# weifengliu-ssslab/Benchmark_SpMV_using_CSR5

Hardware: AMD Instinct MI355X
Metric: fp64 SpMV GFLOPS (higher is better)
Workload: dtype f64

## Files before the change

benchmark_spmv_using_csr5_amd/csrc/csr5_capi.hip:

```cpp
#include <algorithm>
#include <chrono>
#include <cstdio>
#include <cstdlib>
#include <cstring>
#include <string>
#include <unordered_map>
#include <vector>

#include "csr5_internal.h"

using namespace csr5;

namespace {

thread_local std::string g_last_error;

}

namespace csr5 {
void set_last_error(const std::string &msg) { g_last_error = msg; }
}

namespace {

// ... 668 lines not shown
    if (rc != CSR5HIP_SUCCESS)
        return rc;
    Geometry &g = h->g;
    hipStream_t s = h->stream;

    double t0 = now_ms();
    rc = reserve_aux(h);
    if (rc != CSR5HIP_SUCCESS)
        return rc;
    h->t_malloc += now_ms() - t0;

    if (g.p > 0) {
        rc = build_format_arrays(h);
        if (rc != CSR5HIP_SUCCESS)
            return rc;
        if (h->is_child && h->hot_enabled)
            HIP_TRY(launch_transpose_values(g, h->d, h->value_type, s));
        else
            HIP_TRY(launch_transpose(g, h->d, h->value_type, true, s));
        auto finish = [&]() -> int {
            return derive_kernel_tables(h);
        };
        rc = finish();
        if (rc != CSR5HIP_SUCCESS) {
            const std::string why = g_last_error;
            if (h->is_child && h->hot_enabled)
                h->format = -1;
            else if (launch_transpose(g, h->d, h->value_type, false, s) != hipSuccess ||
                     hipStreamSynchronize(s) != hipSuccess)
                h->format = -1;
            g_last_error = why;
            return rc;
        }
// ... 219 lines not shown
        if (!hot && auto_count) {
            if (h->hot_cover_pct >= HOT_AUTO_MIN_COVER_PCT) {
                h->t_slab = now_ms() - t0;
                return CSR5HIP_SUCCESS;
            }
            S = S_plain;
        }
    }
    int bits = 0;
    while ((1 << bits) < S)
        bits++;

    HIP_TRY(h->b_col2.reserve((size_t)g.nnz * 4));
    HIP_TRY(h->b_val2.reserve((size_t)g.nnz * h->vsize()));
    HIP_TRY(slab_partition(g, h->d, h->value_type, S, bits, h->slab_shift, (uint32_t *)t.hist, t.scan_tmp, scan_bytes,
                           (int32_t *)h->b_col2.ptr, h->b_val2.ptr, (uint32_t *)t.key, s));
    HIP_TRY(slab_count_segments(g.nnz, (const uint32_t *)t.key, t.sel_tmp, (unsigned int *)t.count, s));
    unsigned int m2 = 0;
    HIP_TRY(hipMemcpyAsync(&m2, t.count, 4, hipMemcpyDeviceToHost, s));
    HIP_TRY(hipStreamSynchronize(s));
    HIP_TRY(h->b_row_ptr2.reserve(((size_t)m2 + 1) * 4));
    HIP_TRY(h->b_rowidx.reserve((size_t)m2 + 1));
    HIP_TRY(slab_segments(g.nnz, (const uint32_t *)t.key, t.sel_tmp, (int32_t *)h->b_row_ptr2.ptr, (unsigned char *)h->b_rowidx.ptr, s));
    HIP_TRY(h->b_base.reserve(slab_base_words(g.m, S) * 4));
    HIP_TRY(h->b_nonempty.reserve(((size_t)g.m / 32 + 16) * 4));
    HIP_TRY(slab_tables(g.m, (int)m2, g.nnz, S, g.p, h->d.row_ptr, (int32_t *)h->b_row_ptr2.ptr, (const uint32_t *)t.key,
                        (const uint32_t *)t.hist, (uint32_t *)h->b_base.ptr, (uint32_t *)h->b_nonempty.ptr, s));
    HIP_TRY(h->b_P.reserve(((size_t)m2 + 1) * h->vsize()));
    HIP_TRY(hipMemsetAsync(h->b_P.ptr, 0, ((size_t)m2 + 1) * h->vsize(), s));

    if (hot) {
        HIP_TRY(slab_hot_finish(S, g.p, hot_p, hot_T, g.nnz, hot_capacity, (const uint32_t *)t.hist,
                                (int32_t *)h->b_hot_count.ptr, (int32_t *)h->b_hot_tile0.ptr, (int32_t *)h->b_slab_off.ptr, s));
        std::vector<int32_t> first_tile((size_t)S + 1);
        HIP_TRY(hipMemcpyAsync(first_tile.data(), h->b_hot_tile0.ptr, ((size_t)S + 1) * 4, hipMemcpyDeviceToHost, s));
        HIP_TRY(hipStreamSynchronize(s));
        const int rounds = S / NUM_XCD;
        std::vector<int> by_size((size_t)S), order((size_t)S, 0), used(NUM_XCD, 0);
// ... 2 lines not shown
            by_size[k] = k;
        std::stable_sort(by_size.begin(), by_size.end(), [&](int a, int b) {
            return first_tile[a + 1] - first_tile[a] > first_tile[b + 1] - first_tile[b];
        });
        for (int k : by_size) {
            int best = -1;
            for (int x = 0; x < NUM_XCD; x++)
                if (used[x] < rounds && (best < 0 || load[x] < load[best]))
                    best = x;
            order[(size_t)best * rounds + used[best]++] = k;
            load[best] += first_tile[k + 1] - first_tile[k];
        }
        HIP_TRY(hipMemcpyAsync((int32_t *)h->b_hot_tile0.ptr + S + 1, order.data(), (size_t)S * 4, hipMemcpyHostToDevice, s));
        int32_t cold_total = 0;
        {
            HIP_TRY(h->b_col_lo.reserve((size_t)g.nnz * 2 + 64));
            HIP_TRY(h->b_col_hi.reserve((size_t)g.nnz + 64));
            const size_t cold_cap = std::min(cold_words, (size_t)g.nnz);
            HIP_TRY(h->b_cold_base.reserve(((size_t)S + 1) * 4));
            HIP_TRY(h->b_cold_cols.reserve((cold_cap + 1) * 4));
            HIP_TRY(h->b_xperm.reserve(((size_t)S * hot_capacity + cold_cap + (size_t)hot_T + 1) * h->vsize()));
            HIP_TRY(hipMemsetAsync(tb + o_ref, 0, cold_words, s));
            HIP_TRY(slab_hot_pack(g.n, g.nnz, hot_T, hot_p, S, bits, h->slab_shift, (const int32_t *)h->b_slab_off.ptr, ht.hotmap,
                                  (const uint32_t *)ht.cnt, (const uint32_t *)t.key, (int32_t *)h->b_col2.ptr, (uint16_t *)h->b_col_lo.ptr,
                                  (uint8_t *)h->b_col_hi.ptr, (uint8_t *)(tb + o_ref), (uint32_t *)(tb + o_rank),
                                  (uint32_t *)(tb + o_keys), (uint32_t *)(tb + o_keys2),
                                  (uint32_t *)(tb + o_src), tb + o_sort, cold_sort_bytes, (int32_t *)h->b_cold_base.ptr,
                                  (int32_t *)h->b_cold_cols.ptr, s));
            HIP_TRY(hipMemcpyAsync(&cold_total, (int32_t *)h->b_cold_base.ptr + S, 4, hipMemcpyDeviceToHost, s));
        }
        HIP_TRY(hipStreamSynchronize(s));
        h->cold_total = cold_total;
    }
    HIP_TRY(hipStreamSynchronize(s));

    csr5hip_handle c = h->slab_child ? h->slab_child : new csr5hip_handle_s();
    h->slab_child = c;
    c->is_child = true;
    c->g.m = (int)m2;
// ... 720 lines not shown
    return CSR5HIP_SUCCESS;
}

int csr5hip_timer_stop(csr5hip_handle h, double *ms)
{
    if (!h || !ms || !h->ev0)
        return CSR5HIP_INVALID_ARGUMENT;
    HIP_TRY(hipEventRecord(h->ev1, h->stream));
    HIP_TRY(hipEventSynchronize(h->ev1));
    float f = 0;
    HIP_TRY(hipEventElapsedTime(&f, h->ev0, h->ev1));
    *ms = f;
    return CSR5HIP_SUCCESS;
}

}
```

benchmark_spmv_using_csr5_amd/csrc/csr5_format.hip:

```cpp
#include "csr5_internal.h"

#include <rocprim/device/device_scan.hpp>

namespace csr5 {

__device__ __forceinline__ int upper_bound(const int32_t *__restrict__ a, int key, int size)
{
    int lo = 0, hi = size;
    while (lo < hi) {
        int mid = (int)(((unsigned)lo + (unsigned)hi) >> 1);
        if (a[mid] <= key)
            lo = mid + 1;
        else
            hi = mid;
    }
    return lo;
}

__device__ __forceinline__ void stamp_phase(uint32_t *__restrict__ counters, int slot)
{
    if (counters && blockIdx.x == 0 && threadIdx.x == 0)
        *reinterpret_cast<unsigned long long *>(counters + STAMP_WORD + 2 * slot) = wall_clock64();
}

// ... 607 lines not shown
        hipLaunchKernelGGL(k_offset_scan_small, dim3(1), dim3(1024), 0, s, d.offset_ptr, g.p + 1);
        return hipGetLastError();
    }
    return rocprim::exclusive_scan(tmp, tmp_bytes, d.offset_ptr, d.offset_ptr, 0, (size_t)g.p + 1, rocprim::plus<int32_t>(), s);
}

hipError_t launch_desc_offset(const Geometry &g, const DeviceArrays &d, hipStream_t s)
{
    if (g.p <= 1)
        return hipSuccess;
    hipLaunchKernelGGL(k_desc_offset, dim3(div_up(g.p - 1, FMT_WAVES_PER_BLOCK)), dim3(FMT_BLOCK), 0, s, g,
                       d.row_ptr, d.tile_ptr, d.tile_desc, d.offset_ptr, d.offset);
    return hipGetLastError();
}

template <typename VT, int SIGMA>
__global__ void __launch_bounds__(FMT_BLOCK) k_transpose_values(Geometry g, VT *__restrict__ val, uint32_t *__restrict__ counters)
{
    stamp_phase(counters, 2);
    constexpr int T = OMEGA * SIGMA;
    const int lane = threadIdx.x & (OMEGA - 1);
    const int t = blockIdx.x * FMT_WAVES_PER_BLOCK + (threadIdx.x >> 6);
    if (t >= g.p - 1)
        return;
    VT *tile = val + (size_t)t * T;
    VT v[SIGMA];
    constexpr int PER = 16 / sizeof(VT);
    typedef VT piece_t __attribute__((ext_vector_type(PER)));
    static_assert(SIGMA % PER == 0, "whole 16-byte pieces per lane");
#pragma unroll
    for (int q = 0; q < SIGMA / PER; q++) {
        const piece_t w = *reinterpret_cast<const piece_t *>(tile + lane * SIGMA + q * PER);
#pragma unroll
        for (int e = 0; e < PER; e++)
            v[q * PER + e] = w[e];
    }
    asm volatile("s_waitcnt vmcnt(0)" ::: "memory");
#pragma unroll
    for (int q = 0; q < SIGMA / PER; q++) {
        piece_t w;
#pragma unroll
        for (int e = 0; e < PER; e++)
            w[e] = v[q * PER + e];
        *reinterpret_cast<piece_t *>(tile + ((size_t)q * OMEGA + lane) * PER) = w;
    }
}

hipError_t launch_transpose(const Geometry &g, const DeviceArrays &d, int value_type, bool r2c, hipStream_t s)
{
    if (g.p <= 1)
        return hipSuccess;
    const size_t vsz = value_type == CSR5HIP_F64 ? 8 : 4;
    int tpb = (int)(12288 / ((size_t)g.tile_elems * (vsz + 4)));
    tpb = tpb < 1 ? 1 : (tpb > 16 ? 16 : tpb);
    const size_t lds = (size_t)tpb * g.sigma * transpose_pitch(g.sigma) * (vsz + 4);
    const dim3 grid((unsigned)((g.p - 1 + tpb - 1) / tpb));
    if (value_type == CSR5HIP_F64)
        hipLaunchKernelGGL(k_transpose<double>, grid, dim3(FMT_BLOCK), lds, s, g, d.tile_ptr, d.col, (double *)d.val, r2c ? 1 : 0, tpb,
                           r2c ? d.counters : nullptr);
    else
        hipLaunchKernelGGL(k_transpose<float>, grid, dim3(FMT_BLOCK), lds, s, g, d.tile_ptr, d.col, (float *)d.val, r2c ? 1 : 0, tpb,
                           r2c ? d.counters : nullptr);
    return hipGetLastError();
}

hipError_t launch_transpose_values(const Geometry &g, const DeviceArrays &d, int value_type, hipStream_t s)
{
    if (g.p <= 1)
        return hipSuccess;
    const dim3 grid((unsigned)div_up(g.p - 1, FMT_WAVES_PER_BLOCK)), block(FMT_BLOCK);
#define CSR5_TV(VT, S)                                                                                                \
    hipLaunchKernelGGL((k_transpose_values<VT, S>), grid, block, 0, s, g, (VT *)d.val, d.counters);                  \
    return hipGetLastError();
    if (value_type == CSR5HIP_F64) {
        switch (g.sigma) {
        case 8: CSR5_TV(double, 8)
        case 16: CSR5_TV(double, 16)
        }
    } else {
        switch (g.sigma) {
        case 8: CSR5_TV(float, 8)
        case 16: CSR5_TV(float, 16)
        }
    }
#undef CSR5_TV
    return hipErrorInvalidValue;
}

hipError_t launch_tile_tables(const Geometry &g, const DeviceArrays &d, int value_size, uint32_t *host_words, bool export_only,
                              hipStream_t s)
{
    if (g.p <= 0)
        return hipSuccess;
    if (export_only) {
        hipLaunchKernelGGL(k_stats_export, dim3(1), dim3(1024), 0, s, g, d.tile_ptr, d.tile_hdr, d.offset_ptr, d.counters,
                           host_words, 1);
        return hipGetLastError();
    }
    hipLaunchKernelGGL(k_tile_tables, dim3(div_up(g.p, FMT_WAVES_PER_BLOCK)), dim3(FMT_BLOCK), 0, s, g, d.row_ptr,
                       d.tile_ptr, d.col, reinterpret_cast<uint4 *>(d.carry_meta), d.tile_hdr, d.counters,
                       xwin_elems(value_size), value_size == 8 ? 4 : 5);
    hipError_t e = hipGetLastError();
    if (e != hipSuccess)
// ... 25 lines not shown
```

benchmark_spmv_using_csr5_amd/csrc/csr5_internal.h:

```cpp
#pragma once

#include <hip/hip_runtime.h>
#include <stdint.h>

#include "csr5hip.h"

namespace csr5 {

constexpr int OMEGA = CSR5HIP_OMEGA;
#ifndef CSR5_WAVES_PER_BLOCK
#define CSR5_WAVES_PER_BLOCK 1
#endif
constexpr int WAVES_PER_BLOCK = CSR5_WAVES_PER_BLOCK;
constexpr int BLOCK = OMEGA * WAVES_PER_BLOCK;
constexpr int FMT_WAVES_PER_BLOCK = 2;
constexpr int FMT_BLOCK = OMEGA * FMT_WAVES_PER_BLOCK;
constexpr int BIT_SS = 6;
constexpr uint32_t ROW_MASK = 0x7FFFFFFFu;
constexpr int STAMP_WORD = 8;
constexpr int COUNTER_WORDS = 16;
constexpr int NUM_XCD = 8;
constexpr int RUN_SERIAL_MAX = 64;
#ifndef CSR5_XWIN_BYTES
#define CSR5_XWIN_BYTES 4096
// ... 49 lines not shown
    const int32_t *cold_cols;
    int cold_total;
    const float *val32;
    const uint32_t *col16;
    const int32_t *base16;
    const uint32_t *col31;
};

hipError_t launch_row_scan(const Geometry &g, const DeviceArrays &d, hipStream_t s);
hipError_t launch_tile_desc(const Geometry &g, const DeviceArrays &d, hipStream_t s);
size_t offset_scan_tmp_bytes(int entries);
hipError_t launch_offset_scan(const Geometry &g, const DeviceArrays &d, void *tmp, size_t tmp_bytes, hipStream_t s);
hipError_t launch_desc_offset(const Geometry &g, const DeviceArrays &d, hipStream_t s);
hipError_t launch_transpose(const Geometry &g, const DeviceArrays &d, int value_type, bool r2c,
                            hipStream_t s);
hipError_t launch_transpose_values(const Geometry &g, const DeviceArrays &d, int value_type, hipStream_t s);
hipError_t launch_tile_tables(const Geometry &g, const DeviceArrays &d, int value_size, uint32_t *host_words, bool export_only,
                              hipStream_t s);
hipError_t launch_col16(const Geometry &g, const DeviceArrays &d, uint32_t *col16, int32_t *base16, uint32_t *wide_tiles,
                        hipStream_t s);
constexpr int COL16_SPAN = 32768;
constexpr bool col16_sigma(int sigma) { return sigma == 8 || sigma == 12 || sigma == 16 || sigma == 24 || sigma == 32; }
hipError_t launch_col31(const Geometry &g, const DeviceArrays &d, uint32_t *col31, hipStream_t s);
constexpr bool col31_sigma(int sigma) { return sigma >= 4 && sigma <= 8; }
hipError_t launch_warmup(hipStream_t s);
hipError_t launch_validate_csr(int m, int n, int nnz, const int32_t *row_ptr, const int32_t *col, uint32_t *flag,
                               hipStream_t s);

hipError_t slab_scan_tmp_bytes(size_t items, size_t *bytes);
hipError_t slab_select_tmp_bytes(int nnz, size_t *bytes);
hipError_t slab_partition(const Geometry &g, const DeviceArrays &d, int value_type, int S, int bits, int shift,
                          uint32_t *hist, void *scan_tmp, size_t scan_tmp_bytes, int32_t *col2, void *val2,
                          uint32_t *key2, hipStream_t s);
hipError_t slab_count_segments(int nnz, const uint32_t *key2, void *tmp, unsigned int *d_count, hipStream_t s);
hipError_t slab_segments(int nnz, const uint32_t *key2, const void *tmp, int32_t *row_ptr2, unsigned char *rowidx, hipStream_t s);
size_t slab_base_words(int m, int S);
hipError_t slab_tables(int m, int m2, int nnz, int S, int p, const int32_t *row_ptr, int32_t *row_ptr2, const uint32_t *key2,
                       const uint32_t *chunk_start, uint32_t *base, uint32_t *nonempty, hipStream_t s);
hipError_t slab_hot_select(int n, int nnz, int S, int bits, int shift, int capacity, int min_count, int sample_stride,
                           const int32_t *col, uint32_t *cnt, void *hotmap, uint32_t *chist, uint32_t *thr,
                           int32_t *hot_cols, int32_t *hot_count, unsigned long long *covered, hipStream_t s);
hipError_t slab_hot_finish(int S, int p_hist, int p, int T, int nnz, int capacity, const uint32_t *chunk_start,
                           int32_t *hot_count, int32_t *tile0, int32_t *slab_off, hipStream_t s);
size_t slab_cold_words(int n, int S, int bits, int shift);
hipError_t slab_cold_sort_tmp_bytes(size_t total, int slab_bits, size_t *bytes);
hipError_t slab_hot_pack(int n, int nnz, int T, int p, int S, int bits, int shift, const int32_t *slab_off, const void *hotmap,
                         const uint32_t *cnt, const uint32_t *key2, int32_t *col2, uint16_t *col_lo, uint8_t *col_hi, uint8_t *ref, uint32_t *rank_of,
                         uint32_t *keys, uint32_t *keys_sorted, uint32_t *src_sorted, void *sort_tmp, size_t sort_tmp_bytes,
                         int32_t *cold_base, int32_t *cold_cols, hipStream_t s);
size_t slab_local_columns(int n, int bits, int shift);
size_t slab_hotmap_bytes(int n, int S, int bits, int shift);
int slab_hot_buckets();
hipError_t launch_slab_combine(int m, int tail_start, int zero_empty, int S, int value_type, const uint32_t *base,
                               const unsigned char *rowidx, const uint32_t *nonempty, const void *P, int segments, void *y,
                               hipStream_t s);

struct SpmvOptions {
    int mode;
    int xcd_remap;
    int x_window;
    int lds_y;
    int stream_nt;
// ... 48 lines not shown
```

benchmark_spmv_using_csr5_amd/csrc/csr5_slab.hip:

```cpp
#include "csr5_internal.h"
#include "csr5_slabmap.h"

#include <rocprim/device/device_radix_sort.hpp>
#include <rocprim/device/device_scan.hpp>
#include <rocprim/iterator/counting_iterator.hpp>

namespace csr5 {

constexpr int SLAB_BLOCK = 256;
constexpr int SLAB_MAX = 64;
constexpr uint32_t SLAB_KEY_FIRST = 0x80000000u;

__host__ __device__ inline size_t slab_hot_groups(int n, int shift, int bits) { return (slab_local_count(n, shift, bits) + 127) / 128; }
__device__ __forceinline__ bool hot_lookup(const uint4 w, uint32_t bit, uint32_t &below)
{
    const unsigned long long lo = (unsigned long long)w.x | ((unsigned long long)w.y << 32);
    const unsigned long long hi = (unsigned long long)w.z | ((unsigned long long)w.w << 32);
    const unsigned long long word = bit < 64 ? lo : hi;
    const uint32_t b = bit & 63;
    below = (uint32_t)__popcll(word & ((1ull << b) - 1ull)) + (bit < 64 ? 0u : (uint32_t)__popcll(lo));
    return (word >> b) & 1ull;
}

__device__ __forceinline__ int upper_bound_i32(const int32_t *__restrict__ a, int key, int size)
// ... 59 lines not shown
    }
}

__device__ __forceinline__ unsigned long long same_slab_lanes(int k, bool valid, int bits)
{
    unsigned long long same = __ballot(valid);
    for (int b = 0; b < bits; b++) {
        const bool on = (k >> b) & 1;
        const unsigned long long bal = __ballot(on);
        same &= on ? bal : ~bal;
    }
    return same;
}

template <typename VT>
__global__ void __launch_bounds__(SLAB_BLOCK)
k_slab_scatter(Geometry g, const int32_t *__restrict__ row_ptr, const uint32_t *__restrict__ tile_ptr,
               const int32_t *__restrict__ col, const VT *__restrict__ val, int S, int bits, int shift,
               const uint32_t *__restrict__ chunk_start, int32_t *__restrict__ col2, VT *__restrict__ val2,
               uint32_t *__restrict__ key2)
{
    extern __shared__ __attribute__((aligned(16))) char smem[];
    const int T = g.tile_elems;
    VT *sval = reinterpret_cast<VT *>(smem);
    int32_t *scol = reinterpret_cast<int32_t *>(smem + (size_t)T * sizeof(VT));
    uint32_t *off = reinterpret_cast<uint32_t *>(smem + (size_t)T * (sizeof(VT) + 4));
    uint16_t *inv = reinterpret_cast<uint16_t *>(off + (size_t)(T / OMEGA) * S);
    unsigned char *skey = reinterpret_cast<unsigned char *>(inv + T);
    unsigned char *srank = skey + T;
    constexpr int ROWCAP = 1024;
    __shared__ int32_t srow[ROWCAP];
    __shared__ uint32_t slab_first[SLAB_MAX], gstart[SLAB_MAX], lstart[SLAB_MAX + 1];

    const int t = blockIdx.x;
    const int tid = threadIdx.x, lane = tid & (OMEGA - 1), wave = tid >> 6;
// ... 50 lines not shown
            lstart[k + 1] += lstart[k];
    }
    __syncthreads();
    for (int c = tid; c < E; c += SLAB_BLOCK) {
        const int k = skey[c];
        inv[lstart[k] + off[(c >> 6) * S + k] + srank[c]] = (uint16_t)c;
    }
    __syncthreads();
    for (int o = tid; o < E; o += SLAB_BLOCK) {
        const int c = inv[o];
        const int k = skey[c];
        const size_t dst = (size_t)gstart[k] + ((uint32_t)o - lstart[k]);
        const int j = (int)(base + c);
        const int row = rs + (rows_in_lds ? upper_bound_i32(srow, j, re - rs) : upper_bound_i32(row_ptr + rs + 1, j, re - rs));
        col2[dst] = scol[c];
        val2[dst] = sval[c];
        key2[dst] = (uint32_t)row | (dst == slab_first[k] ? SLAB_KEY_FIRST : 0u);
    }
}

__device__ __forceinline__ bool key_starts(uint32_t a, uint32_t before)
{
    return (a & SLAB_KEY_FIRST) != 0 || ((a ^ before) & ~SLAB_KEY_FIRST) != 0;
}
__device__ __forceinline__ unsigned segment_starts4(const uint32_t *__restrict__ key, long long j, long long hi, uint32_t k[4])
{
    if (j >= hi)
        return 0u;
    const uint32_t before = j > 0 ? key[j - 1] : 0u;
    if (j + 4 <= hi) {
        const uint4 v = *reinterpret_cast<const uint4 *>(key + j);
// ... 75 lines not shown
    for (int k = 0; k < w; k++)
        run += wave_total[k];
    for (int i = 0; i < per; i++)
        if (first + i < blocks) {
            block_count[first + i] = run;
            run += v[i];
        }
    if (threadIdx.x == 1023) {
        block_count[blocks] = run;
        *total = run;
    }
}

__global__ void __launch_bounds__(SLAB_BLOCK)
k_slab_emit_segments(int nnz, const uint32_t *__restrict__ key, const unsigned int *__restrict__ block_offset,
                     int32_t *__restrict__ row_ptr2, unsigned char *__restrict__ rowidx)
{
    __shared__ unsigned wave_count[SLAB_BLOCK / OMEGA];
    const long long chunk = seg_chunk(nnz, gridDim.x);
    const long long lo = (long long)blockIdx.x * chunk, hi = lo + chunk < nnz ? lo + chunk : nnz;
    const int lane = threadIdx.x & (OMEGA - 1), w = threadIdx.x / OMEGA;
    unsigned out = block_offset[blockIdx.x];
    for (long long j0 = lo; j0 < hi; j0 += SEG_STEP) {
        const long long j = j0 + (long long)threadIdx.x * 4;
        uint32_t k4[4];
        const unsigned f = segment_starts4(key, j, hi, k4);
        const unsigned own = (unsigned)__popc(f);
        unsigned incl = own;
#pragma unroll
        for (int d = 1; d < OMEGA; d <<= 1) {
            const unsigned o = __shfl_up(incl, d, OMEGA);
            if (lane >= d)
                incl += o;
        }
        if (lane == OMEGA - 1)
            wave_count[w] = incl;
        __syncthreads();
        unsigned before = 0, all = 0;
        for (int k = 0; k < SLAB_BLOCK / OMEGA; k++) {
            before += k < w ? wave_count[k] : 0u;
            all += wave_count[k];
        }
        unsigned at = out + before + incl - own;
#pragma unroll
        for (int i = 0; i < 4; i++)
            if (f & (1u << i)) {
                row_ptr2[at] = (int32_t)(j + i);
                rowidx[at++] = (unsigned char)(k4[i] & (COMBINE_ROWS - 1));
            }
        out += all;
        __syncthreads();
    }
}

__global__ void __launch_bounds__(SLAB_BLOCK)
k_slab_base(int m2, int nnz, int S, int nblk, const int32_t *__restrict__ row_ptr2, const uint32_t *__restrict__ key,
            const uint32_t *__restrict__ chunk_start, int p, uint32_t *__restrict__ base, int32_t *__restrict__ row_ptr2_end)
{
// ... 448 lines not shown
                slot++;
            }
        }
    }
    if (blockIdx.y == gridDim.y - 1 && threadIdx.x == 0)
        hot_count[k] = (int32_t)(running + all);
}

constexpr int ENCODE_BLOCK = 1024, ENCODE_WGS_PER_XCD = 32, ENCODE_UNROLL = 4;
constexpr int ENC_MARK = 1, ENC_PACK = 2;
template <bool IN_LDS, int MODE>
__global__ void __launch_bounds__(ENCODE_BLOCK)
k_hot_encode(int nnz, int T, int p, int S, int bits, int shift, const int32_t *__restrict__ slab_off,
             const uint4 *__restrict__ hotbits, const uint16_t *__restrict__ hotpre, size_t G, int32_t *__restrict__ col2,
             uint16_t *__restrict__ col_lo, uint8_t *__restrict__ col_hi, uint8_t *__restrict__ ref,
             const uint32_t *__restrict__ rank_of, size_t L, const uint32_t *__restrict__ key)
{
    extern __shared__ __attribute__((aligned(16))) char smem[];
    uint4 *lbits = reinterpret_cast<uint4 *>(smem);
    uint16_t *lpre = reinterpret_cast<uint16_t *>(smem + G * sizeof(uint4));
    __shared__ int32_t soff[SLAB_MAX + 1];
    if ((int)threadIdx.x <= S)
        soff[threadIdx.x] = slab_off[threadIdx.x];
    __syncthreads();
    const int xcd = blockIdx.x % NUM_XCD, j = blockIdx.x / NUM_XCD, nj = gridDim.x / NUM_XCD;
    const long long last = (long long)(p - 1) * T;
    for (int mine = xcd; mine < S; mine += NUM_XCD) {
        const uint4 *gb = hotbits + (size_t)mine * G;
        const uint16_t *gp = hotpre + (size_t)mine * G;
        if (IN_LDS) {
            __syncthreads();
// ... 41 lines not shown
            for (int u = 0; u < ENCODE_UNROLL; u++) {
                const long long q = q0 + u * ENCODE_BLOCK + threadIdx.x;
                if (q < quads)
                    v[u] = c4[q];
            }
#pragma unroll
            for (int u = 0; u < ENCODE_UNROLL; u++) {
                const long long q = q0 + u * ENCODE_BLOCK + threadIdx.x;
                if (q < quads) {
                    const long long pos = begin + q * 4;
                    v[u].x = encode(v[u].x, pos);
                    v[u].y = encode(v[u].y, pos + 1);
                    v[u].z = encode(v[u].z, pos + 2);
                    v[u].w = encode(v[u].w, pos + 3);
                    if (MODE == ENC_PACK) {
                        uint32_t k4[4];
                        const unsigned st = segment_starts4(key, pos, (long long)nnz, k4);
                        const uint32_t a = (uint32_t)v[u].x | ((st & 1u) << 22), b = (uint32_t)v[u].y | (((st >> 1) & 1u) << 22),
                                       c = (uint32_t)v[u].z | (((st >> 2) & 1u) << 22), d = (uint32_t)v[u].w | (((st >> 3) & 1u) << 22);
                        lo4[q] = make_uint2((a & 0xFFFFu) | (b << 16), (c & 0xFFFFu) | (d << 16));
                        hi4[q] = ((a >> 16) & 0xFFu) | (((b >> 16) & 0xFFu) << 8) | (((c >> 16) & 0xFFu) << 16) | ((d >> 16) << 24);
                    }
                }
            }
        }
    }
}

constexpr uint32_t COLD_COUNT_CAP = 1023, COLD_KEY_BITS = 11;
__global__ void __launch_bounds__(SLAB_BLOCK)
k_cold_keys(size_t total, size_t L, int n, int bits, int shift, const uint8_t *__restrict__ ref, const uint32_t *__restrict__ cnt,
            uint32_t *__restrict__ keys)
{
    const size_t i = (size_t)blockIdx.x * SLAB_BLOCK + threadIdx.x;
    if (i >= total)
        return;
// ... 46 lines not shown
    if ((int32_t)r >= cold_base[k + 1] - b)
        return;
    const uint32_t src = src_sorted[q];
    rank_of[src] = r;
    cold_cols[(size_t)b + r] = (int32_t)slab_column(k, (uint32_t)(src - (size_t)k * L), shift, bits);
}

size_t slab_scatter_lds(const Geometry &g, int S, size_t vsize)
{
    const size_t T = (size_t)g.tile_elems;
    return T * (vsize + 4) + (T / OMEGA) * (size_t)S * 4 + T * 2 + T + T;
}

hipError_t slab_partition(const Geometry &g, const DeviceArrays &d, int value_type, int S, int bits, int shift,
                          uint32_t *hist, void *scan_tmp, size_t scan_tmp_bytes, int32_t *col2, void *val2,
                          uint32_t *key2, hipStream_t s)
{
    const size_t hist_lds = (size_t)(SLAB_BLOCK / OMEGA) * S * HIST_PAD * 4;
    hipError_t e = hipFuncSetAttribute(reinterpret_cast<const void *>(k_slab_hist), hipFuncAttributeMaxDynamicSharedMemorySize,
                                       (int)hist_lds);
    if (e != hipSuccess)
        return e;
    hipLaunchKernelGGL(k_slab_hist, dim3((g.p + HIST_TILES - 1) / HIST_TILES), dim3(SLAB_BLOCK), hist_lds, s, g, d.col, S, bits, shift,
                       hist);
    e = hipGetLastError();
    if (e != hipSuccess)
        return e;
    e = rocprim::exclusive_scan(scan_tmp, scan_tmp_bytes, hist, hist, 0u, (size_t)S * g.p, rocprim::plus<uint32_t>(), s);
    if (e != hipSuccess)
        return e;
    const size_t vs = value_type == CSR5HIP_F64 ? 8 : 4;
    const size_t lds = slab_scatter_lds(g, S, vs);
    if (value_type == CSR5HIP_F64)
        hipLaunchKernelGGL(k_slab_scatter<double>, dim3(g.p), dim3(SLAB_BLOCK), lds, s, g, d.row_ptr, d.tile_ptr, d.col,
                           (const double *)d.val, S, bits, shift, hist, col2, (double *)val2, key2);
    else
        hipLaunchKernelGGL(k_slab_scatter<float>, dim3(g.p), dim3(SLAB_BLOCK), lds, s, g, d.row_ptr, d.tile_ptr, d.col,
                           (const float *)d.val, S, bits, shift, hist, col2, (float *)val2, key2);
    return hipGetLastError();
}

hipError_t slab_scan_tmp_bytes(size_t items, size_t *bytes)
{
    uint32_t *null_u = nullptr;
    return rocprim::exclusive_scan(nullptr, *bytes, null_u, null_u, 0u, items, rocprim::plus<uint32_t>(), nullptr);
}

hipError_t slab_select_tmp_bytes(int nnz, size_t *bytes)
{
    *bytes = ((size_t)seg_blocks(nnz) + 1) * 4;
    return hipSuccess;
}

hipError_t slab_count_segments(int nnz, const uint32_t *key2, void *tmp, unsigned int *d_count, hipStream_t s)
{
    const int blocks = seg_blocks(nnz);
    hipLaunchKernelGGL(k_slab_count_segments, dim3(blocks), dim3(SLAB_BLOCK), 0, s, nnz, key2, (unsigned int *)tmp);
    hipLaunchKernelGGL(k_slab_scan_counts, dim3(1), dim3(1024), 0, s, blocks, (unsigned int *)tmp, d_count);
    return hipGetLastError();
}

hipError_t slab_segments(int nnz, const uint32_t *key2, const void *tmp, int32_t *row_ptr2, unsigned char *rowidx, hipStream_t s)
{
    hipLaunchKernelGGL(k_slab_emit_segments, dim3(seg_blocks(nnz)), dim3(SLAB_BLOCK), 0, s, nnz, key2,
                       (const unsigned int *)tmp, row_ptr2, rowidx);
    return hipGetLastError();
}

size_t slab_base_words(int m, int S) { return ((size_t)(m + COMBINE_ROWS - 1) / COMBINE_ROWS + 2) * (size_t)S; }
hipError_t slab_tables(int m, int m2, int nnz, int S, int p, const int32_t *row_ptr, int32_t *row_ptr2, const uint32_t *key2,
                       const uint32_t *chunk_start, uint32_t *base, uint32_t *nonempty, hipStream_t s)
{
    const int nblk = (m + COMBINE_ROWS - 1) / COMBINE_ROWS;
    const long long entries = (long long)(nblk + 1) * S;
    hipLaunchKernelGGL(k_slab_base, dim3((unsigned)((entries + SLAB_BLOCK - 1) / SLAB_BLOCK)), dim3(SLAB_BLOCK), 0, s, m2, nnz, S,
                       nblk, row_ptr2, key2, chunk_start, p, base, row_ptr2 + m2);
    hipLaunchKernelGGL(k_slab_nonempty, dim3((m + 32 + SLAB_BLOCK - 1) / SLAB_BLOCK), dim3(SLAB_BLOCK), 0, s, m, row_ptr, nonempty);
    return hipGetLastError();
}

// ... 70 lines not shown
    hipLaunchKernelGGL(k_hot_rank, dim3(S, (unsigned)((G + RANK_BLOCK - 1) / RANK_BLOCK)), dim3(RANK_BLOCK), 0, s, bits, shift,
                       capacity, G, hotbits, hotpre, hot_cols, hot_count);
    return hipGetLastError();
}

hipError_t slab_hot_finish(int S, int p_hist, int p, int T, int nnz, int capacity, const uint32_t *chunk_start,
                           int32_t *hot_count, int32_t *tile0, int32_t *slab_off, hipStream_t s)
{
    hipLaunchKernelGGL(k_hot_finish, dim3(1), dim3(SLAB_MAX + 1), 0, s, S, p_hist, p, T, nnz, capacity, chunk_start,
                       hot_count, tile0, slab_off);
    return hipGetLastError();
}

static hipError_t hot_encode_pass(int mode, int n, int nnz, int T, int p, int S, int bits, int shift, const int32_t *slab_off,
                                  const void *hotmap, int32_t *col2, uint16_t *col_lo, uint8_t *col_hi, uint8_t *ref,
                                  const uint32_t *rank_of, const uint32_t *key, hipStream_t s)
{
    const size_t G = slab_hot_groups(n, shift, bits);
    const size_t L = slab_local_count(n, shift, bits);
    const uint4 *hotbits = (const uint4 *)hotmap;
    const uint16_t *hotpre = (const uint16_t *)(hotbits + (size_t)S * G);
    const size_t lds = G * (sizeof(uint4) + sizeof(uint16_t));
    const dim3 grid(NUM_XCD * ENCODE_WGS_PER_XCD), block(ENCODE_BLOCK);
    const bool in_lds = lds <= 150 * 1024;
    auto launch = [&](auto kern) -> hipError_t {
        if (in_lds) {
            hipError_t e = hipFuncSetAttribute(reinterpret_cast<const void *>(kern), hipFuncAttributeMaxDynamicSharedMemorySize,
                                               (int)lds);
            if (e != hipSuccess)
                return e;
        }
        hipLaunchKernelGGL(kern, grid, block, in_lds ? lds : 0, s, nnz, T, p, S, bits, shift, slab_off, hotbits, hotpre, G, col2,
                           col_lo, col_hi, ref, rank_of, L, key);
        return hipGetLastError();
    };
    if (mode == ENC_MARK)
        return in_lds ? launch(k_hot_encode<true, ENC_MARK>) : launch(k_hot_encode<false, ENC_MARK>);
    return in_lds ? launch(k_hot_encode<true, ENC_PACK>) : launch(k_hot_encode<false, ENC_PACK>);
}

size_t slab_cold_words(int n, int S, int bits, int shift) { return (size_t)S * slab_local_count(n, shift, bits); }
hipError_t slab_cold_sort_tmp_bytes(size_t total, int slab_bits, size_t *bytes)
{
    uint32_t *nu = nullptr;
    rocprim::counting_iterator<uint32_t> iota(0u);
    return rocprim::radix_sort_pairs(nullptr, *bytes, nu, nu, iota, nu, total, 0, slab_bits + (int)COLD_KEY_BITS, nullptr);
}

hipError_t slab_hot_pack(int n, int nnz, int T, int p, int S, int bits, int shift, const int32_t *slab_off, const void *hotmap,
                         const uint32_t *cnt, const uint32_t *key2, int32_t *col2, uint16_t *col_lo, uint8_t *col_hi, uint8_t *ref, uint32_t *rank_of,
                         uint32_t *keys, uint32_t *keys_sorted, uint32_t *src_sorted, void *sort_tmp, size_t sort_tmp_bytes,
                         int32_t *cold_base, int32_t *cold_cols, hipStream_t s)
{
    const size_t L = slab_local_count(n, shift, bits), total = (size_t)S * L;
    hipError_t e = hot_encode_pass(ENC_MARK, n, nnz, T, p, S, bits, shift, slab_off, hotmap, col2, nullptr, nullptr, ref, nullptr, nullptr, s);
    if (e != hipSuccess)
        return e;
    const unsigned blocks = (unsigned)((total + SLAB_BLOCK - 1) / SLAB_BLOCK);
    hipLaunchKernelGGL(k_cold_keys, dim3(blocks), dim3(SLAB_BLOCK), 0, s, total, L, n, bits, shift, ref, cnt, keys);
    rocprim::counting_iterator<uint32_t> iota(0u);
    e = rocprim::radix_sort_pairs(sort_tmp, sort_tmp_bytes, keys, keys_sorted, iota, src_sorted, total, 0, bits + (int)COLD_KEY_BITS, s);
    if (e != hipSuccess)
        return e;
    hipLaunchKernelGGL(k_cold_layout, dim3(1), dim3(SLAB_MAX), 0, s, S, L, keys_sorted, cold_base);
    hipLaunchKernelGGL(k_cold_rank, dim3(blocks), dim3(SLAB_BLOCK), 0, s, total, L, bits, shift, src_sorted, cold_base, rank_of, cold_cols);
    e = hipGetLastError();
    if (e != hipSuccess)
        return e;
    return hot_encode_pass(ENC_PACK, n, nnz, T, p, S, bits, shift, slab_off, hotmap, col2, col_lo, col_hi, nullptr, rank_of, key2, s);
}

size_t slab_local_columns(int n, int bits, int shift) { return slab_local_count(n, shift, bits); }

size_t slab_hotmap_bytes(int n, int S, int bits, int shift)
{
    return (size_t)S * slab_hot_groups(n, shift, bits) * (sizeof(uint4) + sizeof(uint16_t)) + 256;
}

int slab_hot_buckets() { return HOT_BUCKETS; }

}
```

Measured before the change: 485.6.

## Fuse value transpose into slab scatter and precompute segment-start bits in segment emit

The slab scatter kernel now writes values directly into the child's transposed tile layout, so the separate in-place value transpose kernel is removed. Segment-start flags for the hot encoding are written into col_hi by the segment-emit kernel rather than recomputed from keys during the pack pass. Both changes touch only the preprocessing/format-build path, reducing passes over values and keys there. A debug digest function is added to check the resulting arrays.

```diff
diff --git a/benchmark_spmv_using_csr5_amd/csrc/csr5_capi.hip b/benchmark_spmv_using_csr5_amd/csrc/csr5_capi.hip
--- a/benchmark_spmv_using_csr5_amd/csrc/csr5_capi.hip
+++ b/benchmark_spmv_using_csr5_amd/csrc/csr5_capi.hip
@@ -706,9 +706,7 @@
         rc = build_format_arrays(h);
         if (rc != CSR5HIP_SUCCESS)
             return rc;
-        if (h->is_child && h->hot_enabled)
-            HIP_TRY(launch_transpose_values(g, h->d, h->value_type, s));
-        else
+        if (!(h->is_child && h->hot_enabled))
             HIP_TRY(launch_transpose(g, h->d, h->value_type, true, s));
         auto finish = [&]() -> int {
             return derive_kernel_tables(h);
@@ -958,14 +956,19 @@
     HIP_TRY(h->b_col2.reserve((size_t)g.nnz * 4));
     HIP_TRY(h->b_val2.reserve((size_t)g.nnz * h->vsize()));
     HIP_TRY(slab_partition(g, h->d, h->value_type, S, bits, h->slab_shift, (uint32_t *)t.hist, t.scan_tmp, scan_bytes,
-                           (int32_t *)h->b_col2.ptr, h->b_val2.ptr, (uint32_t *)t.key, s));
+                           (int32_t *)h->b_col2.ptr, h->b_val2.ptr, (uint32_t *)t.key, hot ? hot_T : 0, hot ? hot_p - 1 : 0, s));
     HIP_TRY(slab_count_segments(g.nnz, (const uint32_t *)t.key, t.sel_tmp, (unsigned int *)t.count, s));
     unsigned int m2 = 0;
     HIP_TRY(hipMemcpyAsync(&m2, t.count, 4, hipMemcpyDeviceToHost, s));
     HIP_TRY(hipStreamSynchronize(s));
     HIP_TRY(h->b_row_ptr2.reserve(((size_t)m2 + 1) * 4));
     HIP_TRY(h->b_rowidx.reserve((size_t)m2 + 1));
-    HIP_TRY(slab_segments(g.nnz, (const uint32_t *)t.key, t.sel_tmp, (int32_t *)h->b_row_ptr2.ptr, (unsigned char *)h->b_rowidx.ptr, s));
+    if (hot) {
+        HIP_TRY(h->b_col_lo.reserve((size_t)g.nnz * 2 + 64));
+        HIP_TRY(h->b_col_hi.reserve((size_t)g.nnz + 64));
+    }
+    HIP_TRY(slab_segments(g.nnz, (const uint32_t *)t.key, t.sel_tmp, (int32_t *)h->b_row_ptr2.ptr, (unsigned char *)h->b_rowidx.ptr,
+                          hot ? (uint8_t *)h->b_col_hi.ptr : nullptr, s));
     HIP_TRY(h->b_base.reserve(slab_base_words(g.m, S) * 4));
     HIP_TRY(h->b_nonempty.reserve(((size_t)g.m / 32 + 16) * 4));
     HIP_TRY(slab_tables(g.m, (int)m2, g.nnz, S, g.p, h->d.row_ptr, (int32_t *)h->b_row_ptr2.ptr, (const uint32_t *)t.key,
@@ -998,15 +1001,13 @@
         HIP_TRY(hipMemcpyAsync((int32_t *)h->b_hot_tile0.ptr + S + 1, order.data(), (size_t)S * 4, hipMemcpyHostToDevice, s));
         int32_t cold_total = 0;
         {
-            HIP_TRY(h->b_col_lo.reserve((size_t)g.nnz * 2 + 64));
-            HIP_TRY(h->b_col_hi.reserve((size_t)g.nnz + 64));
             const size_t cold_cap = std::min(cold_words, (size_t)g.nnz);
             HIP_TRY(h->b_cold_base.reserve(((size_t)S + 1) * 4));
             HIP_TRY(h->b_cold_cols.reserve((cold_cap + 1) * 4));
             HIP_TRY(h->b_xperm.reserve(((size_t)S * hot_capacity + cold_cap + (size_t)hot_T + 1) * h->vsize()));
             HIP_TRY(hipMemsetAsync(tb + o_ref, 0, cold_words, s));
             HIP_TRY(slab_hot_pack(g.n, g.nnz, hot_T, hot_p, S, bits, h->slab_shift, (const int32_t *)h->b_slab_off.ptr, ht.hotmap,
-                                  (const uint32_t *)ht.cnt, (const uint32_t *)t.key, (int32_t *)h->b_col2.ptr, (uint16_t *)h->b_col_lo.ptr,
+                                  (const uint32_t *)ht.cnt, (int32_t *)h->b_col2.ptr, (uint16_t *)h->b_col_lo.ptr,
                                   (uint8_t *)h->b_col_hi.ptr, (uint8_t *)(tb + o_ref), (uint32_t *)(tb + o_rank),
                                   (uint32_t *)(tb + o_keys), (uint32_t *)(tb + o_keys2),
                                   (uint32_t *)(tb + o_src), tb + o_sort, cold_sort_bytes, (int32_t *)h->b_cold_base.ptr,
@@ -1757,4 +1758,56 @@
     return CSR5HIP_SUCCESS;
 }
 
-}
+int csr5hip_debug_slab_digest(csr5hip_handle h, unsigned long long *out, int count)
+{
+    if (!h || !out || h->slab_S <= 0 || !h->slab_child)
+        return CSR5HIP_INVALID_ARGUMENT;
+    const csr5hip_handle_s *c = h->slab_child;
+    const int S = h->slab_S;
+    const size_t nnz = (size_t)h->g.nnz, m2 = (size_t)h->slab_m2, vs = h->vsize();
+    const bool hot = c->hot_enabled;
+    const size_t body = hot && c->g.p > 1 ? (size_t)(c->g.p - 1) * c->g.tile_elems : 0;
+    HIP_TRY(hipStreamSynchronize(h->stream));
+    struct Part {
+        const void *p;
+        size_t bytes;
+    } arrays[] = {
+        {h->b_col2.ptr, nnz * 4},
+        {h->b_val2.ptr, nnz * vs},
+        {h->b_row_ptr2.ptr, (m2 + 1) * 4},
+        {h->b_rowidx.ptr, m2},
+        {h->b_base.ptr, ((size_t)(h->g.m + 255) / 256 + 1) * S * 4},
+        {h->b_nonempty.ptr, ((size_t)h->g.m + 31) / 32 * 4},
+        {hot ? h->b_col_lo.ptr : nullptr, body * 2},
+        {hot ? h->b_col_hi.ptr : nullptr, body},
+        {hot ? h->b_cold_base.ptr : nullptr, ((size_t)S + 1) * 4},
+        {hot ? h->b_cold_cols.ptr : nullptr, (size_t)h->cold_total * 4},
+        {hot ? h->b_hot_cols.ptr : nullptr, (size_t)S * c->d.hot_capacity * 4},
+        {hot ? h->b_hot_count.ptr : nullptr, (size_t)S * 4},
+        {hot ? h->b_hot_tile0.ptr : nullptr, ((size_t)2 * S + 1) * 4},
+        {hot ? h->b_slab_off.ptr : nullptr, ((size_t)S + 1) * 4},
+        {hot ? h->b_range_head.ptr : nullptr, ((size_t)S * HOT_RANGES_PER_SLAB + 1) * 4},
+        {h->values_narrowed ? h->b_val32.ptr : nullptr, nnz * 4},
+    };
+    const unsigned long long head[6] = {(unsigned long long)S, m2, hot ? 1ull : 0ull, (unsigned long long)h->cold_total,
+                                        h->values_narrowed ? 1ull : 0ull, (unsigned long long)c->g.p};
+    int w = 0;
+    for (unsigned long long v : head)
+        if (w < count)
+            out[w++] = v;
+    std::vector<unsigned char> host;
+    for (const Part &a : arrays) {
+        unsigned long long f = 0xcbf29ce484222325ull;
+        if (a.p && a.bytes) {
+            host.resize(a.bytes);
+            HIP_TRY(hipMemcpy(host.data(), a.p, a.bytes, hipMemcpyDeviceToHost));
+            for (unsigned char b : host)
+                f = (f ^ b) * 0x100000001b3ull;
+        }
+        if (w < count)
+            out[w++] = f;
+    }
+    return w;
+}
+
+}
diff --git a/benchmark_spmv_using_csr5_amd/csrc/csr5_format.hip b/benchmark_spmv_using_csr5_amd/csrc/csr5_format.hip
--- a/benchmark_spmv_using_csr5_amd/csrc/csr5_format.hip
+++ b/benchmark_spmv_using_csr5_amd/csrc/csr5_format.hip
@@ -645,38 +645,6 @@
     return hipGetLastError();
 }
 
-template <typename VT, int SIGMA>
-__global__ void __launch_bounds__(FMT_BLOCK) k_transpose_values(Geometry g, VT *__restrict__ val, uint32_t *__restrict__ counters)
-{
-    stamp_phase(counters, 2);
-    constexpr int T = OMEGA * SIGMA;
-    const int lane = threadIdx.x & (OMEGA - 1);
-    const int t = blockIdx.x * FMT_WAVES_PER_BLOCK + (threadIdx.x >> 6);
-    if (t >= g.p - 1)
-        return;
-    VT *tile = val + (size_t)t * T;
-    VT v[SIGMA];
-    constexpr int PER = 16 / sizeof(VT);
-    typedef VT piece_t __attribute__((ext_vector_type(PER)));
-    static_assert(SIGMA % PER == 0, "whole 16-byte pieces per lane");
-#pragma unroll
-    for (int q = 0; q < SIGMA / PER; q++) {
-        const piece_t w = *reinterpret_cast<const piece_t *>(tile + lane * SIGMA + q * PER);
-#pragma unroll
-        for (int e = 0; e < PER; e++)
-            v[q * PER + e] = w[e];
-    }
-    asm volatile("s_waitcnt vmcnt(0)" ::: "memory");
-#pragma unroll
-    for (int q = 0; q < SIGMA / PER; q++) {
-        piece_t w;
-#pragma unroll
-        for (int e = 0; e < PER; e++)
-            w[e] = v[q * PER + e];
-        *reinterpret_cast<piece_t *>(tile + ((size_t)q * OMEGA + lane) * PER) = w;
-    }
-}
-
 hipError_t launch_transpose(const Geometry &g, const DeviceArrays &d, int value_type, bool r2c, hipStream_t s)
 {
     if (g.p <= 1)
@@ -695,29 +663,6 @@
     return hipGetLastError();
 }
 
-hipError_t launch_transpose_values(const Geometry &g, const DeviceArrays &d, int value_type, hipStream_t s)
-{
-    if (g.p <= 1)
-        return hipSuccess;
-    const dim3 grid((unsigned)div_up(g.p - 1, FMT_WAVES_PER_BLOCK)), block(FMT_BLOCK);
-#define CSR5_TV(VT, S)                                                                                                \
-    hipLaunchKernelGGL((k_transpose_values<VT, S>), grid, block, 0, s, g, (VT *)d.val, d.counters);                  \
-    return hipGetLastError();
-    if (value_type == CSR5HIP_F64) {
-        switch (g.sigma) {
-        case 8: CSR5_TV(double, 8)
-        case 16: CSR5_TV(double, 16)
-        }
-    } else {
-        switch (g.sigma) {
-        case 8: CSR5_TV(float, 8)
-        case 16: CSR5_TV(float, 16)
-        }
-    }
-#undef CSR5_TV
-    return hipErrorInvalidValue;
-}
-
 hipError_t launch_tile_tables(const Geometry &g, const DeviceArrays &d, int value_size, uint32_t *host_words, bool export_only,
                               hipStream_t s)
 {
diff --git a/benchmark_spmv_using_csr5_amd/csrc/csr5_internal.h b/benchmark_spmv_using_csr5_amd/csrc/csr5_internal.h
--- a/benchmark_spmv_using_csr5_amd/csrc/csr5_internal.h
+++ b/benchmark_spmv_using_csr5_amd/csrc/csr5_internal.h
@@ -87,7 +87,6 @@
 hipError_t launch_desc_offset(const Geometry &g, const DeviceArrays &d, hipStream_t s);
 hipError_t launch_transpose(const Geometry &g, const DeviceArrays &d, int value_type, bool r2c,
                             hipStream_t s);
-hipError_t launch_transpose_values(const Geometry &g, const DeviceArrays &d, int value_type, hipStream_t s);
 hipError_t launch_tile_tables(const Geometry &g, const DeviceArrays &d, int value_size, uint32_t *host_words, bool export_only,
                               hipStream_t s);
 hipError_t launch_col16(const Geometry &g, const DeviceArrays &d, uint32_t *col16, int32_t *base16, uint32_t *wide_tiles,
@@ -104,9 +103,10 @@
 hipError_t slab_select_tmp_bytes(int nnz, size_t *bytes);
 hipError_t slab_partition(const Geometry &g, const DeviceArrays &d, int value_type, int S, int bits, int shift,
                           uint32_t *hist, void *scan_tmp, size_t scan_tmp_bytes, int32_t *col2, void *val2,
-                          uint32_t *key2, hipStream_t s);
+                          uint32_t *key2, int child_tile, int child_body_tiles, hipStream_t s);
 hipError_t slab_count_segments(int nnz, const uint32_t *key2, void *tmp, unsigned int *d_count, hipStream_t s);
-hipError_t slab_segments(int nnz, const uint32_t *key2, const void *tmp, int32_t *row_ptr2, unsigned char *rowidx, hipStream_t s);
+hipError_t slab_segments(int nnz, const uint32_t *key2, const void *tmp, int32_t *row_ptr2, unsigned char *rowidx,
+                         uint8_t *start_hi, hipStream_t s);
 size_t slab_base_words(int m, int S);
 hipError_t slab_tables(int m, int m2, int nnz, int S, int p, const int32_t *row_ptr, int32_t *row_ptr2, const uint32_t *key2,
                        const uint32_t *chunk_start, uint32_t *base, uint32_t *nonempty, hipStream_t s);
@@ -118,7 +118,7 @@
 size_t slab_cold_words(int n, int S, int bits, int shift);
 hipError_t slab_cold_sort_tmp_bytes(size_t total, int slab_bits, size_t *bytes);
 hipError_t slab_hot_pack(int n, int nnz, int T, int p, int S, int bits, int shift, const int32_t *slab_off, const void *hotmap,
-                         const uint32_t *cnt, const uint32_t *key2, int32_t *col2, uint16_t *col_lo, uint8_t *col_hi, uint8_t *ref, uint32_t *rank_of,
+                         const uint32_t *cnt, int32_t *col2, uint16_t *col_lo, uint8_t *col_hi, uint8_t *ref, uint32_t *rank_of,
                          uint32_t *keys, uint32_t *keys_sorted, uint32_t *src_sorted, void *sort_tmp, size_t sort_tmp_bytes,
                          int32_t *cold_base, int32_t *cold_cols, hipStream_t s);
 size_t slab_local_columns(int n, int bits, int shift);
diff --git a/benchmark_spmv_using_csr5_amd/csrc/csr5_slab.hip b/benchmark_spmv_using_csr5_amd/csrc/csr5_slab.hip
--- a/benchmark_spmv_using_csr5_amd/csrc/csr5_slab.hip
+++ b/benchmark_spmv_using_csr5_amd/csrc/csr5_slab.hip
@@ -97,11 +97,21 @@
 }
 
 template <typename VT>
+__device__ __forceinline__ size_t piece_position(size_t dst, int vshift)
+{
+    constexpr uint32_t PER = 16 / sizeof(VT);
+    const size_t t0 = dst >> vshift << vshift;
+    const uint32_t r = (uint32_t)(dst - t0), sshift = (uint32_t)vshift - 6;
+    const uint32_t l = r >> sshift, e = r & ((1u << sshift) - 1u);
+    return t0 + (size_t)(((e / PER) * OMEGA + l) * PER + e % PER);
+}
+
+template <typename VT>
 __global__ void __launch_bounds__(SLAB_BLOCK)
 k_slab_scatter(Geometry g, const int32_t *__restrict__ row_ptr, const uint32_t *__restrict__ tile_ptr,
                const int32_t *__restrict__ col, const VT *__restrict__ val, int S, int bits, int shift,
                const uint32_t *__restrict__ chunk_start, int32_t *__restrict__ col2, VT *__restrict__ val2,
-               uint32_t *__restrict__ key2)
+               uint32_t *__restrict__ key2, int vshift, size_t vbody)
 {
     extern __shared__ __attribute__((aligned(16))) char smem[];
     const int T = g.tile_elems;
@@ -182,7 +192,7 @@
         const int j = (int)(base + c);
         const int row = rs + (rows_in_lds ? upper_bound_i32(srow, j, re - rs) : upper_bound_i32(row_ptr + rs + 1, j, re - rs));
         col2[dst] = scol[c];
-        val2[dst] = sval[c];
+        val2[dst < vbody ? piece_position<VT>(dst, vshift) : dst] = sval[c];
         key2[dst] = (uint32_t)row | (dst == slab_first[k] ? SLAB_KEY_FIRST : 0u);
     }
 }
@@ -288,7 +298,7 @@
 
 __global__ void __launch_bounds__(SLAB_BLOCK)
 k_slab_emit_segments(int nnz, const uint32_t *__restrict__ key, const unsigned int *__restrict__ block_offset,
-                     int32_t *__restrict__ row_ptr2, unsigned char *__restrict__ rowidx)
+                     int32_t *__restrict__ row_ptr2, unsigned char *__restrict__ rowidx, uint32_t *__restrict__ start_hi)
 {
     __shared__ unsigned wave_count[SLAB_BLOCK / OMEGA];
     const long long chunk = seg_chunk(nnz, gridDim.x);
@@ -316,6 +326,8 @@
             all += wave_count[k];
         }
         unsigned at = out + before + incl - own;
+        if (start_hi && j < hi)
+            start_hi[j >> 2] = ((f & 1u) << 6) | ((f & 2u) << 13) | ((f & 4u) << 20) | ((f & 8u) << 27);
 #pragma unroll
         for (int i = 0; i < 4; i++)
             if (f & (1u << i)) {
@@ -794,7 +806,7 @@
 k_hot_encode(int nnz, int T, int p, int S, int bits, int shift, const int32_t *__restrict__ slab_off,
              const uint4 *__restrict__ hotbits, const uint16_t *__restrict__ hotpre, size_t G, int32_t *__restrict__ col2,
              uint16_t *__restrict__ col_lo, uint8_t *__restrict__ col_hi, uint8_t *__restrict__ ref,
-             const uint32_t *__restrict__ rank_of, size_t L, const uint32_t *__restrict__ key)
+             const uint32_t *__restrict__ rank_of, size_t L)
 {
     extern __shared__ __attribute__((aligned(16))) char smem[];
     uint4 *lbits = reinterpret_cast<uint4 *>(smem);
@@ -866,12 +878,10 @@
                     v[u].z = encode(v[u].z, pos + 2);
                     v[u].w = encode(v[u].w, pos + 3);
                     if (MODE == ENC_PACK) {
-                        uint32_t k4[4];
-                        const unsigned st = segment_starts4(key, pos, (long long)nnz, k4);
-                        const uint32_t a = (uint32_t)v[u].x | ((st & 1u) << 22), b = (uint32_t)v[u].y | (((st >> 1) & 1u) << 22),
-                                       c = (uint32_t)v[u].z | (((st >> 2) & 1u) << 22), d = (uint32_t)v[u].w | (((st >> 3) & 1u) << 22);
+                        const uint32_t st = hi4[q];
+                        const uint32_t a = (uint32_t)v[u].x, b = (uint32_t)v[u].y, c = (uint32_t)v[u].z, d = (uint32_t)v[u].w;
                         lo4[q] = make_uint2((a & 0xFFFFu) | (b << 16), (c & 0xFFFFu) | (d << 16));
-                        hi4[q] = ((a >> 16) & 0xFFu) | (((b >> 16) & 0xFFu) << 8) | (((c >> 16) & 0xFFu) << 16) | ((d >> 16) << 24);
+                        hi4[q] = st | ((a >> 16) & 0xFFu) | (((b >> 16) & 0xFFu) << 8) | (((c >> 16) & 0xFFu) << 16) | ((d >> 16) << 24);
                     }
                 }
             }
@@ -948,8 +958,14 @@
 
 hipError_t slab_partition(const Geometry &g, const DeviceArrays &d, int value_type, int S, int bits, int shift,
                           uint32_t *hist, void *scan_tmp, size_t scan_tmp_bytes, int32_t *col2, void *val2,
-                          uint32_t *key2, hipStream_t s)
-{
+                          uint32_t *key2, int child_tile, int child_body_tiles, hipStream_t s)
+{
+    int vshift = 0;
+    while (child_tile > 0 && (1 << vshift) < child_tile)
+        vshift++;
+    if (child_tile > 0 && ((1 << vshift) != child_tile || vshift < 6 + (value_type == CSR5HIP_F64 ? 1 : 2)))
+        return hipErrorInvalidValue;
+    const size_t vbody = child_tile > 0 && child_body_tiles > 0 ? (size_t)child_body_tiles * (size_t)child_tile : 0;
     const size_t hist_lds = (size_t)(SLAB_BLOCK / OMEGA) * S * HIST_PAD * 4;
     hipError_t e = hipFuncSetAttribute(reinterpret_cast<const void *>(k_slab_hist), hipFuncAttributeMaxDynamicSharedMemorySize,
                                        (int)hist_lds);
@@ -967,10 +983,10 @@
     const size_t lds = slab_scatter_lds(g, S, vs);
     if (value_type == CSR5HIP_F64)
         hipLaunchKernelGGL(k_slab_scatter<double>, dim3(g.p), dim3(SLAB_BLOCK), lds, s, g, d.row_ptr, d.tile_ptr, d.col,
-                           (const double *)d.val, S, bits, shift, hist, col2, (double *)val2, key2);
+                           (const double *)d.val, S, bits, shift, hist, col2, (double *)val2, key2, vshift, vbody);
     else
         hipLaunchKernelGGL(k_slab_scatter<float>, dim3(g.p), dim3(SLAB_BLOCK), lds, s, g, d.row_ptr, d.tile_ptr, d.col,
-                           (const float *)d.val, S, bits, shift, hist, col2, (float *)val2, key2);
+                           (const float *)d.val, S, bits, shift, hist, col2, (float *)val2, key2, vshift, vbody);
     return hipGetLastError();
 }
 
@@ -994,10 +1010,11 @@
     return hipGetLastError();
 }
 
-hipError_t slab_segments(int nnz, const uint32_t *key2, const void *tmp, int32_t *row_ptr2, unsigned char *rowidx, hipStream_t s)
+hipError_t slab_segments(int nnz, const uint32_t *key2, const void *tmp, int32_t *row_ptr2, unsigned char *rowidx,
+                         uint8_t *start_hi, hipStream_t s)
 {
     hipLaunchKernelGGL(k_slab_emit_segments, dim3(seg_blocks(nnz)), dim3(SLAB_BLOCK), 0, s, nnz, key2,
-                       (const unsigned int *)tmp, row_ptr2, rowidx);
+                       (const unsigned int *)tmp, row_ptr2, rowidx, (uint32_t *)start_hi);
     return hipGetLastError();
 }
 
@@ -1098,7 +1115,7 @@
 
 static hipError_t hot_encode_pass(int mode, int n, int nnz, int T, int p, int S, int bits, int shift, const int32_t *slab_off,
                                   const void *hotmap, int32_t *col2, uint16_t *col_lo, uint8_t *col_hi, uint8_t *ref,
-                                  const uint32_t *rank_of, const uint32_t *key, hipStream_t s)
+                                  const uint32_t *rank_of, hipStream_t s)
 {
     const size_t G = slab_hot_groups(n, shift, bits);
     const size_t L = slab_local_count(n, shift, bits);
@@ -1115,7 +1132,7 @@
                 return e;
         }
         hipLaunchKernelGGL(kern, grid, block, in_lds ? lds : 0, s, nnz, T, p, S, bits, shift, slab_off, hotbits, hotpre, G, col2,
-                           col_lo, col_hi, ref, rank_of, L, key);
+                           col_lo, col_hi, ref, rank_of, L);
         return hipGetLastError();
     };
     if (mode == ENC_MARK)
@@ -1132,12 +1149,12 @@
 }
 
 hipError_t slab_hot_pack(int n, int nnz, int T, int p, int S, int bits, int shift, const int32_t *slab_off, const void *hotmap,
-                         const uint32_t *cnt, const uint32_t *key2, int32_t *col2, uint16_t *col_lo, uint8_t *col_hi, uint8_t *ref, uint32_t *rank_of,
+                         const uint32_t *cnt, int32_t *col2, uint16_t *col_lo, uint8_t *col_hi, uint8_t *ref, uint32_t *rank_of,
                          uint32_t *keys, uint32_t *keys_sorted, uint32_t *src_sorted, void *sort_tmp, size_t sort_tmp_bytes,
                          int32_t *cold_base, int32_t *cold_cols, hipStream_t s)
 {
     const size_t L = slab_local_count(n, shift, bits), total = (size_t)S * L;
-    hipError_t e = hot_encode_pass(ENC_MARK, n, nnz, T, p, S, bits, shift, slab_off, hotmap, col2, nullptr, nullptr, ref, nullptr, nullptr, s);
+    hipError_t e = hot_encode_pass(ENC_MARK, n, nnz, T, p, S, bits, shift, slab_off, hotmap, col2, nullptr, nullptr, ref, nullptr, s);
     if (e != hipSuccess)
         return e;
     const unsigned blocks = (unsigned)((total + SLAB_BLOCK - 1) / SLAB_BLOCK);
@@ -1151,7 +1168,7 @@
     e = hipGetLastError();
     if (e != hipSuccess)
         return e;
-    return hot_encode_pass(ENC_PACK, n, nnz, T, p, S, bits, shift, slab_off, hotmap, col2, col_lo, col_hi, nullptr, rank_of, key2, s);
+    return hot_encode_pass(ENC_PACK, n, nnz, T, p, S, bits, shift, slab_off, hotmap, col2, col_lo, col_hi, nullptr, rank_of, s);
 }
 
 size_t slab_local_columns(int n, int bits, int shift) { return slab_local_count(n, shift, bits); }
```

Measured after the change: 485.6, median of 4. About the same (-0.0%).
